# RRr89/Shared_SIMD_Scan

Measured on AMD Instinct MI355X. Metric: scanned values/sec + achieved HBM GB/s, 1e9 x 9-bit column (equality scan, bitmap + hit count out), higher is better.
Workload: dtype u32; 1 GPU; scan_eq ONE 1e+09x9bit column in 1 row-range shard(s) of <= 1000000000 rows, column=mod5, key=3; rows_total=1000000000, bits=9, parallelism=row-range shards x1

## Files before the change

shared_simd_scan_amd/csrc/kernels/in_list.hpp:

```cpp
#pragma once

#include "scan.hpp"

namespace mi355 {

template <int C, int AUX_, int VPL>
__global__ __launch_bounds__(kBlockThreads) void in_kernel(ScanArgs a)
{
    using G = ScanGeom<C, VPL>;
    constexpr int WORDS = G::WORDS;
    constexpr int AUX = AUX_ & 15;
    constexpr int NTS = store_policy_of(AUX_);
    constexpr bool BITSET = C <= 16;
    constexpr int SET_BYTES = BITSET ? ((1 << (C < 16 ? C : 16)) + 7) / 8 : 16;
    __shared__ __attribute__((aligned(16))) uint8_t lds[kWavesPerBlock][G::LDS_BYTES];
    __shared__ __attribute__((aligned(16))) uint32_t set_words[(SET_BYTES + 3) / 4];
    __shared__ __attribute__((aligned(16))) uint8_t mlds[kWavesPerBlock][1024];

    const int lane = threadIdx.x & 63;
    const int wave = __builtin_amdgcn_readfirstlane(threadIdx.x >> 6);
    uint8_t *lds_wave = lds[wave];
    const TileCtx<C, VPL> tc(a.n);
    const uint64_t stride = (uint64_t)gridDim.x * kWavesPerBlock;
    uint64_t tile = (uint64_t)blockIdx.x * kWavesPerBlock + wave;
// ... 69 lines not shown
            for (int j = 0; j < WORDS; j++) res[j] = m[j];
        }
        const uint32_t inv = a.invert;
#pragma unroll
        for (int j = 0; j < WORDS; j++) res[j] ^= inv;
        if (tile < tc.nfull) {
            if (a.and_mask) {
#pragma unroll
                for (int j = 0; j < WORDS; j++) res[j] &= mcur[j];
            }
#pragma unroll
            for (int j = 0; j < WORDS; j++) hits += __builtin_popcount(res[j]);
            prev = tile;
        } else {
            const int64_t left = (int64_t)(tc.n - tile * G::TILE_VALUES) - (int64_t)lane * VPL;
            const int nbytes = left <= 0 ? 0 : (int)((left >= VPL ? VPL : left) + 7) / 8;
            if (a.and_mask) {
                const uint8_t *mp = a.and_mask + tile * G::BITMAP_BYTES + lane * (WORDS * 4);
#pragma unroll
                for (int j = 0; j < WORDS; j++) {
                    uint32_t mm = 0;
#pragma unroll
                    for (int b = 0; b < 4; b++)
                        if (4 * j + b < nbytes) mm |= (uint32_t)mp[4 * j + b] << (8 * b);
                    res[j] &= mm;
                }
            }
            hits += tc.finish_tail(tile, res, out_lane + tile * G::BITMAP_BYTES, 1, lane);
            prev = ~0ull;
        }
        tile = next;
    }
    if (prev != ~0ull) store_words<WORDS, NTS>(out_lane + prev * G::BITMAP_BYTES, res);
    if (a.hits) hits_add(a, 0, wave_sum(hits), lane);
    hits_finalize(a, 1, lane);
}

}
```

shared_simd_scan_amd/csrc/kernels/scan.hpp:

```cpp
#pragma once

#include "tile.hpp"

namespace mi355 {

template <int C, int VPL> struct TileCtx {
    using G = ScanGeom<C, VPL>;
    uint64_t n, ntiles, nfull, data_bytes;
    uint32_t llc_inv, llc_lim;
    __device__ __forceinline__ TileCtx(uint64_t n_, uint32_t llc_inv_ = 0, uint32_t llc_lim_ = 0) : n(n_), llc_inv(llc_inv_), llc_lim(llc_lim_)
    {
        ntiles = (n + G::TILE_VALUES - 1) / G::TILE_VALUES;
        nfull = n / G::TILE_VALUES;
        data_bytes = (n * C + 7) / 8;
    }
    template <int AUX> __device__ __forceinline__ void issue(const uint8_t *packed, uint64_t t, uint8_t *lds_wave, int lane) const
    {
        if constexpr (AUX != 0) {
            if (llc_inv != 0 && (uint32_t)((t * G::TILE_BYTES) >> kLlcGranuleShift) * llc_inv <= llc_lim) {
                issue_as<0>(packed, t, lds_wave, lane);
                return;
            }
        }
        issue_as<AUX>(packed, t, lds_wave, lane);
// ... 172 lines not shown
                    for (int j = 0; j < WORDS; j++) {
                        hits += __builtin_popcount(r1[0][j]);
                        res[k][j] = r1[0][j];
                    }
                    nfull_here = k + 1;
                } else {
                    if (mask) {
                        const uint8_t *mp = mask + tile * G::BITMAP_BYTES + lane * (WORDS * 4);
                        const int64_t left = (int64_t)(tc.n - tile * G::TILE_VALUES) - (int64_t)lane * VPL;
                        const int nbytes = left <= 0 ? 0 : (int)((left >= VPL ? VPL : left) + 7) / 8;
#pragma unroll
                        for (int j = 0; j < WORDS; j++) {
                            uint32_t m = 0;
#pragma unroll
                            for (int b = 0; b < 4; b++)
                                if (4 * j + b < nbytes) m |= (uint32_t)mp[4 * j + b] << (8 * b);
                            r1[0][j] = combine(r1[0][j], m);
                        }
                    }
                    hits += tc.finish_tail(tile, r1[0], out_lane + tile * G::BITMAP_BYTES, 1, lane, store);
                }
            }
        }
        pend_chunk = chunk;
        pend_n = nfull_here;
        chunk += stride;
    }
    if (pend_n && store) {
        uint8_t *dst = out_lane + pend_chunk * K * G::BITMAP_BYTES;
#pragma unroll
        for (int q = 0; q < K; q++)
            if (q < pend_n) store_words<WORDS, NTS>(dst + q * G::BITMAP_BYTES, res[q]);
    }
    if (a.hits) hits_add(a, 0, wave_sum(hits), lane);
    hits_finalize(a, 1, lane);
}

template <int C, int AUX_, int VPL>
__global__ __launch_bounds__(kBlockThreads, (burst_occ<C, VPL, 1>() > 1 ? burst_occ<C, VPL, 1>() / 2 : 1)) void scan2_kernel(ScanArgs a)
{
    using G = ScanGeom<C, VPL>;
    constexpr int WORDS = G::WORDS;
    constexpr int AUX = AUX_ & 15;
    constexpr int NTS = store_policy_of(AUX_);
    __shared__ __attribute__((aligned(16))) uint8_t lds[kWavesPerBlock][2][G::LDS_BYTES];

    const int lane = threadIdx.x & 63;
    const int wave = __builtin_amdgcn_readfirstlane(threadIdx.x >> 6);
    uint8_t *lds1 = lds[wave][0], *lds2 = lds[wave][1];
    const TileCtx<C, VPL> tc(a.n);
    const uint64_t stride = (uint64_t)gridDim.x * kWavesPerBlock;
    uint64_t tile = (uint64_t)blockIdx.x * kWavesPerBlock + wave;
    const uint32_t k1[kMaxKeysPerPass] = {a.key[0], a.key[1], 0, 0, 0, 0, 0, 0};
    const uint32_t k2[kMaxKeysPerPass] = {a.key2[0], a.key2[1], 0, 0, 0, 0, 0, 0};
    const uint32_t inv1 = a.invert, inv2 = a.invert2, mop = a.mask_op;
    auto combine = [mop](uint32_t p2, uint32_t p1) -> uint32_t {
        return mop == 0 ? (p2 & p1) : mop == 1 ? (p2 | p1) : mop == 2 ? (p2 ^ p1) : (p1 & ~p2);
    };
    uint32_t hits = 0;
    uint8_t *const out_lane = a.out + lane * (WORDS * 4);
    const bool store = a.out != nullptr;
    uint32_t res[WORDS];
    uint64_t prev = ~0ull;

    auto issue = [&](uint64_t t) {
        tc.template issue<AUX>(a.packed, t, lds1, lane);
        tc.template issue<AUX>(a.packed2, t, lds2, lane);
    };
    if (tile < tc.ntiles) issue(tile);
    while (tile < tc.ntiles) {
        asm volatile("s_waitcnt vmcnt(0)" ::: "memory");
        uint32_t w1[G::LANE_DWORDS], w2[G::LANE_DWORDS];
        read_lane_data<C, VPL>(lds1, lane, w1);
        read_lane_data<C, VPL>(lds2, lane, w2);
        asm volatile("s_waitcnt lgkmcnt(0)" ::: "memory");
        if (prev != ~0ull && store) store_words<WORDS, NTS>(out_lane + prev * G::BITMAP_BYTES, res);
        const uint64_t next = tile + stride;
        if (next < tc.ntiles) issue(next);
        uint32_t r1[1][WORDS], r2[1][WORDS];
        decode_words<C, VPL, 0, 1, kModeRange, G::LANE_DWORDS>(w1, r1, k1);
        decode_words<C, VPL, 0, 1, kModeRange, G::LANE_DWORDS>(w2, r2, k2);
#pragma unroll
        for (int j = 0; j < WORDS; j++) res[j] = combine(r2[0][j] ^ inv2, r1[0][j] ^ inv1);
        if (tile < tc.nfull) {
#pragma unroll
            for (int j = 0; j < WORDS; j++) hits += __builtin_popcount(res[j]);
            prev = tile;
        } else {
            hits += tc.finish_tail(tile, res, out_lane + tile * G::BITMAP_BYTES, 1, lane, store);
            prev = ~0ull;
        }
        tile = next;
    }
    if (prev != ~0ull && store) store_words<WORDS, NTS>(out_lane + prev * G::BITMAP_BYTES, res);
    if (a.hits) hits_add(a, 0, wave_sum(hits), lane);
    hits_finalize(a, 1, lane);
}

__device__ __forceinline__ void transpose4x4_bytes(const uint32_t (&r)[4], uint32_t (&c)[4])
{
    const uint32_t t0 = __builtin_amdgcn_perm(r[1], r[0], 0x05010400u);
    const uint32_t t1 = __builtin_amdgcn_perm(r[1], r[0], 0x07030602u);
    const uint32_t t2 = __builtin_amdgcn_perm(r[3], r[2], 0x05010400u);
    const uint32_t t3 = __builtin_amdgcn_perm(r[3], r[2], 0x07030602u);
    c[0] = __builtin_amdgcn_perm(t2, t0, 0x05040100u);
    c[1] = __builtin_amdgcn_perm(t2, t0, 0x07060302u);
    c[2] = __builtin_amdgcn_perm(t3, t1, 0x05040100u);
    c[3] = __builtin_amdgcn_perm(t3, t1, 0x07060302u);
}

}
```

shared_simd_scan_amd/csrc/kernels/shared.hpp:

```cpp
#pragma once

#include "scan.hpp"

namespace mi355 {

template <int C, int AUX_, int VPL>
__global__ __launch_bounds__(kBlockThreads) void shared_general_kernel(ScanArgs a)
{
    using G = ScanGeom<C, VPL>;
    constexpr int NK = kMaxKeysPerPass;
    constexpr int WORDS = G::WORDS;
    constexpr int AUX = AUX_ & 15;
    __shared__ __attribute__((aligned(16))) uint8_t lds[kWavesPerBlock][G::LDS_BYTES];
    __shared__ uint32_t s_hits[kMaxKeys];
    block_hits_clear(s_hits);
    __syncthreads();

    const int lane = threadIdx.x & 63;
    const int wave = __builtin_amdgcn_readfirstlane(threadIdx.x >> 6);
    uint8_t *lds_wave = lds[wave];
    const TileCtx<C, VPL> tc(a.n);
    const uint64_t stride = (uint64_t)gridDim.x * kWavesPerBlock;
    uint64_t tile = (uint64_t)blockIdx.x * kWavesPerBlock + wave;
    const uint32_t P = a.nkeys;
// ... 45 lines not shown
#pragma unroll
                        for (int j = 0; j < WORDS; j++) cnt += __builtin_popcount(res[q][j]);
                    }
                    cnts[q] = cnt;
                }
            }
            if (a.hits) block_hits_add8(s_hits, pass * kMaxKeysPerPass, P, cnts, lane);
            if (a.layout != 0 && full) {
                const uint32_t nk = (P - pass * 8) < 8 ? (P - pass * 8) : 8;
                const uint64_t g0 = tile * G::BITMAP_BYTES + (uint64_t)lane * (WORDS * 4);
#pragma unroll
                for (int j = 0; j < WORDS; j++) {
                    const uint32_t r0[4] = {res[0][j], res[1][j], res[2][j], res[3][j]};
                    const uint32_t r1[4] = {res[4][j], res[5][j], res[6][j], res[7][j]};
                    uint32_t c0[4], c1[4];
                    transpose4x4_bytes(r0, c0);
                    transpose4x4_bytes(r1, c1);
#pragma unroll
                    for (int b = 0; b < 4; b++) {
                        uint8_t *dst = a.out + (g0 + 4 * j + b) * P + pass * 8;
                        if (nk == 8) {
                            store8_unaligned(dst, c0[b], c1[b]);
                        } else {
#pragma unroll
                            for (int q = 0; q < 8; q++)
                                if ((uint32_t)q < nk) dst[q] = (uint8_t)((q < 4 ? c0[b] : c1[b]) >> (8 * (q & 3)));
                        }
                    }
                }
            }
        }
        tile = next;
    }
    if (a.hits) block_hits_flush(a, s_hits, P);
    hits_finalize(a, P, lane);
}

template <int C, int AUX_, int VPL>
__global__ __launch_bounds__(kBlockThreads) void shared_pair_kernel(ScanArgs a)
{
    using G = ScanGeom<C, VPL>;
    constexpr int WORDS = G::WORDS;
    constexpr int AUX = AUX_ & 15;
    constexpr int NTS = store_policy_of(AUX_);
    __shared__ __attribute__((aligned(16))) uint8_t lds[kWavesPerBlock][G::LDS_BYTES];
    const int lane = threadIdx.x & 63;
    const int wave = __builtin_amdgcn_readfirstlane(threadIdx.x >> 6);
    uint8_t *lds_wave = lds[wave];
    const TileCtx<C, VPL> tc(a.n);
    const uint64_t stride = (uint64_t)gridDim.x * kWavesPerBlock;
    uint64_t tile = (uint64_t)blockIdx.x * kWavesPerBlock + wave;
    const uint32_t k0 = a.key[0], k1 = a.key[1];
    const bool linear = a.layout != 0;
    uint32_t hits0 = 0, hits1 = 0;

    if (tile < tc.ntiles) tc.template issue<AUX>(a.packed, tile, lds_wave, lane);
    int behind = 0;
    while (tile < tc.ntiles) {
        if (behind == 2)
            asm volatile("s_waitcnt vmcnt(2)" ::: "memory");
        else if (behind == 1)
            asm volatile("s_waitcnt vmcnt(1)" ::: "memory");
        else
            asm volatile("s_waitcnt vmcnt(0)" ::: "memory");
        uint32_t w[G::LANE_DWORDS];
        read_lane_data<C, VPL>(lds_wave, lane, w);
        asm volatile("s_waitcnt lgkmcnt(0)" ::: "memory");
        const uint64_t next = tile + stride;
// ... 8 lines not shown
            for (int j = 0; j < WORDS; j++) {
                hits0 += __builtin_popcount(r0[0][j]);
                hits1 += __builtin_popcount(r1[0][j]);
            }
            if (!linear) {
                uint8_t *dst = a.out + tile * G::BITMAP_BYTES + lane * (WORDS * 4);
                store_words<WORDS, NTS>(dst, r0[0]);
                store_words<WORDS, NTS>(dst + a.out_stride, r1[0]);
                behind = 2;
            } else {
                uint32_t y[2 * WORDS];
#pragma unroll
                for (int j = 0; j < WORDS; j++) {
                    y[2 * j] = __builtin_amdgcn_perm(r1[0][j], r0[0][j], 0x05010400u);
                    y[2 * j + 1] = __builtin_amdgcn_perm(r1[0][j], r0[0][j], 0x07030602u);
                }
                uint8_t *dst = a.out + (tile * G::BITMAP_BYTES + (uint64_t)lane * (WORDS * 4)) * 2;
#pragma unroll
                for (int i = 0; i < 2 * WORDS; i += 4) {
                    const uint32_t v[4] = {y[i], y[i + 1], y[i + 2], y[i + 3]};
                    store_words<4, NTS>(dst + 4 * i, v);
                }
                behind = WORDS / 2;
            }
        } else {
            uint8_t *dst = linear ? a.out + (tile * G::BITMAP_BYTES + (uint64_t)lane * (WORDS * 4)) * 2
                                  : a.out + tile * G::BITMAP_BYTES + lane * (WORDS * 4);
            hits0 += tc.finish_tail(tile, r0[0], dst, linear ? 2 : 1, lane);
            hits1 += tc.finish_tail(tile, r1[0], linear ? dst + 1 : dst + a.out_stride, linear ? 2 : 1, lane);
            behind = 0;
        }
        tile = next;
    }
    if (a.hits) {
        hits_add(a, 0, wave_sum(hits0), lane);
        hits_add(a, 1, wave_sum(hits1), lane);
    }
    hits_finalize(a, 2, lane);
}


struct __attribute__((packed, aligned(1))) Unaligned128 { uint32_t w[4]; };

extern __shared__ __attribute__((aligned(16))) uint8_t mi355_dyn_lds[];

template <int C, bool MULTI> struct LutGeom {
    static constexpr int ND = MULTI ? (C <= 10 ? 1 : (C + 7) / 8) : (C <= 16 ? 1 : (C <= 24 ? 2 : 3));
    static constexpr bool SINGLE = ND == 1;
    static constexpr int DIGIT_BITS = SINGLE ? C : (MULTI ? 8 : (C + ND - 1) / ND);
    static constexpr int ENTRIES = 1 << DIGIT_BITS;
    static constexpr int TABLE_BYTES = ND * ENTRIES;
    static __device__ __forceinline__ uint32_t digit(uint32_t x, int d)
    {
        return (d == ND - 1) ? (x >> (DIGIT_BITS * d)) : ((x >> (DIGIT_BITS * d)) & (uint32_t)(ENTRIES - 1));
    }
};

__device__ __forceinline__ void transpose8x8(uint32_t &lo, uint32_t &hi)
{
    uint32_t t;
    t = (lo ^ (lo >> 7)) & 0x00AA00AAu;  lo ^= t ^ (t << 7);
    t = (hi ^ (hi >> 7)) & 0x00AA00AAu;  hi ^= t ^ (t << 7);
    t = (lo ^ (lo >> 14)) & 0x0000CCCCu; lo ^= t ^ (t << 14);
    t = (hi ^ (hi >> 14)) & 0x0000CCCCu; hi ^= t ^ (t << 14);
    t = (lo ^ ((lo >> 28) | (hi << 4))) & 0xF0F0F0F0u;
    lo ^= t;
    hi ^= t >> 4;
}

template <int C, bool MULTI> __device__ __forceinline__ uint32_t lut_lookup(const uint8_t *table, uint32_t x)
{
// ... 403 lines not shown
                } else {
                    lut_words<C, VPL, true, MULTI>(xs, table, valid, out);
                }
                uint32_t tcnt[8];
#pragma unroll
                for (int q = 0; q < 8; q++) {
                    const uint32_t k = pass * 8 + q;
                    tcnt[q] = 0;
                    if (k < P) {
                        uint32_t cnt = 0;
#pragma unroll
                        for (int j = 0; j < WORDS; j++) cnt += __builtin_popcount(out[q][j]);
                        if constexpr (!MULTI)
                            hits[q] += cnt;
                        else
                            tcnt[q] = cnt;
                        uint8_t *dst = LAYOUT == 0
                                           ? a.out + (uint64_t)k * a.out_stride + tile * G::BITMAP_BYTES + lane * (WORDS * 4)
                                           : a.out + (tile * G::BITMAP_BYTES + (uint64_t)lane * GROUPS) * P + k;
                        const uint64_t bstride = LAYOUT == 0 ? 1 : P;
#pragma unroll
                        for (int b = 0; b < WORDS * 4; b++)
                            if (b < nbytes) dst[(uint64_t)b * bstride] = (uint8_t)(out[q][b >> 2] >> (8 * (b & 3)));
                    }
                }
                if constexpr (MULTI) {
                    if (a.hits) block_hits_add8(s_hits, pass * 8, P, tcnt, lane);
                }
            }
        }
        tile = next;
    }
    if constexpr (MULTI) {
        if (a.hits) block_hits_flush(a, s_hits, P);
    }
    if constexpr (!MULTI) {
        if (prev != ~0ull) {
            if (lin8) {
                u32x4 staged[GROUPS / 2];
                stage_get(staged);
                stage_store(prev, staged);
            } else {
                store_full(prev, 0, resp);
            }
        }
        if (a.hits) {
#pragma unroll
            for (int q = 0; q < 8; q++) {
                uint32_t s = wave_sum(hits[q]);
                if ((uint32_t)q < P) hits_add(a, q, s, lane);
            }
        }
    }
    hits_finalize(a, P, lane);
}

template <int C, bool BIG = false> struct WideLutGeom {
    static constexpr int ND = C <= 10 ? 1 : (BIG && C >= 17 && C <= 20) ? 2 : (BIG && C >= 25 && C <= 30) ? 3 : (C + 7) / 8;
    static constexpr bool SINGLE = ND == 1;
    static constexpr int DIGIT_BITS = SINGLE ? C : (BIG ? (C + ND - 1) / ND : 8);
    static constexpr int ENTRIES = 1 << DIGIT_BITS;
    static constexpr int TABLE_DWORDS = ND * ENTRIES;
    static constexpr int TABLE_BYTES = TABLE_DWORDS * 4;
    static __device__ __forceinline__ uint32_t digit(uint32_t x, int d)
    {
        return (d == ND - 1) ? (x >> (DIGIT_BITS * d)) : ((x >> (DIGIT_BITS * d)) & (uint32_t)(ENTRIES - 1));
    }
    static __device__ __forceinline__ uint32_t lookup(const uint32_t *table, uint32_t x)
    {
        if constexpr (SINGLE) {
            return table[x];
        } else {
            uint32_t m = table[digit(x, 0)];
#pragma unroll
            for (int d = 1; d < ND; d++) m &= table[d * ENTRIES + digit(x, d)];
            return m;
        }
    }
};

__device__ __forceinline__ void wait_dma_behind_stores(uint32_t nstores)
{
    if (nstores >= 48)
        asm volatile("s_waitcnt vmcnt(48)" ::: "memory");
    else if (nstores >= 32)
        asm volatile("s_waitcnt vmcnt(32)" ::: "memory");
    else if (nstores >= 16)
// ... 142 lines not shown
                        }
                        if (a.hits) block_hits_add8(s_hits, pass * 8, P, cnt, lane);
                        if (full) {
                            if constexpr (LAYOUT == 0) {
                                uint8_t *dst = a.out + (uint64_t)(pass * 8) * a.out_stride + tile * G::BITMAP_BYTES + lane * (WORDS * 4);
#pragma unroll
                                for (int q = 0; q < 8; q++) {
                                    if (pass * 8 + q < P) store_words<WORDS, NTS>(dst, out[q]);
                                    dst += a.out_stride;
                                }
                            }
                        } else {
                            const int nbytes = (valid + 7) / 8;
#pragma unroll
                            for (int q = 0; q < 8; q++) {
                                const uint32_t k = pass * 8 + q;
                                if (k < P) {
                                    uint8_t *dst = LAYOUT == 0
                                                       ? a.out + (uint64_t)k * a.out_stride + tile * G::BITMAP_BYTES + lane * (WORDS * 4)
                                                       : a.out + (tile * G::BITMAP_BYTES + (uint64_t)lane * GROUPS) * P + k;
                                    const uint64_t bstride = LAYOUT == 0 ? 1 : P;
#pragma unroll
                                    for (int bb = 0; bb < WORDS * 4; bb++)
                                        if (bb < nbytes) dst[(uint64_t)bb * bstride] = (uint8_t)(out[q][bb >> 2] >> (8 * (bb & 3)));
                                }
                            }
                        }
                    }
                }
            }
        }
        tile = next;
    }
    if (a.hits) block_hits_flush(a, s_hits, P);
    hits_finalize(a, P, lane);
}

constexpr uint32_t kPackedFlushTiles = 512;

template <int C, int AUX_, int VPL, int RC = 0, bool BIG = false>
__global__ __launch_bounds__(kBlockThreads) void shared_wide2_kernel(ScanArgs a)
{
    using G = ScanGeom<C, VPL>;
    using L = WideLutGeom<C, BIG>;
    constexpr bool REGCNT = RC == 1;
    constexpr int WORDS = G::WORDS;
    constexpr int AUX = AUX_ & 15;
    constexpr int NTS = store_policy_of(AUX_);
    __shared__ __attribute__((aligned(16))) uint8_t lds[kWavesPerBlock][G::LDS_BYTES];
    __shared__ uint32_t s_hits[kMaxKeys];
    constexpr bool HIST = C <= 12;
    __shared__ uint32_t hist[HIST ? (1 << C) : 1];
    uint32_t *const lut = (uint32_t *)mi355_dyn_lds;
    block_hits_clear(s_hits);
    if constexpr (HIST)
        for (uint32_t k = threadIdx.x; k < (1u << C); k += kBlockThreads) hist[k] = 0;

    const int lane = threadIdx.x & 63;
    const int wave = __builtin_amdgcn_readfirstlane(threadIdx.x >> 6);
    uint8_t *lds_wave = lds[wave];
    const TileCtx<C, VPL> tc(a.n);
    const uint64_t stride = (uint64_t)gridDim.x * kWavesPerBlock;
    uint64_t tile = (uint64_t)blockIdx.x * kWavesPerBlock + wave;
    const uint32_t P = a.nkeys;
    const uint32_t npass32 = (P + 31) / 32;
    constexpr bool reg_counts = REGCNT;
    const bool use_hist = HIST && P >= 64 && RC == 0;
    uint32_t acc[REGCNT ? 4 : 1][8];
// ... 461 lines not shown
            if (copy_out) image_store(pend_gal, pend_a0, pend_end, iv, ihb, itb);
            pend_end = 0;
            if (staged) {
                const uint32_t first = s * row_step;
                const uint32_t rows_in_step = first >= rows_here ? 0u : (rows_here - first < row_step ? rows_here - first : row_step);
                if (rows_in_step) {
                    pend_gal = step_g0 - step_a0;
                    pend_a0 = step_a0;
                    pend_end = step_a0 + rows_in_step * P;
                }
            }
        }
        asm volatile("s_waitcnt lgkmcnt(0)" ::: "memory");
        const uint64_t next = tile + stride;
        if (next < tc.ntiles) tc.template issue<AUX>(a.packed, next, lds_wave, lane);
        tile = next;
    }
    if (pend_end) {
        u32x4 iv[3];
        uint32_t ihb = 0, itb = 0;
        image_load(pend_a0, pend_end, iv, ihb, itb);
        image_store(pend_gal, pend_a0, pend_end, iv, ihb, itb);
    }
    if (!use_hist && a.hits) flush_counts();
    if constexpr (HIST) {
        if (a.hits && use_hist) {
            __syncthreads();
            for (uint32_t k = threadIdx.x; k < P; k += kBlockThreads) {
                const uint32_t key = (uint32_t)a.keys_dev[k];
                s_hits[k] = (key >> C) == 0 ? hist[key] : 0u;
            }
        }
    }
    if (a.hits) block_hits_flush(a, s_hits, P);
    hits_finalize(a, P, lane);
}

template <int C, int AUX_>
__global__ __launch_bounds__(kBlockThreads) void shared_linear2_kernel(ScanArgs a)
{
    constexpr int VPL = 64;
    using G = ScanGeom<C, VPL>;
    using L = WideLutGeom<C>;
    constexpr int AUX = AUX_ & 15;
    constexpr int ROWS = G::TILE_VALUES / 8;
    constexpr int ROW_DW = (C + 3) / 4;
    constexpr int LOAD_DW = (C + 3 + 3) / 4;
    __shared__ __attribute__((aligned(16))) uint8_t lds[kWavesPerBlock][G::LDS_BYTES + 16];
    __shared__ uint32_t s_hits[kMaxKeys];
    constexpr bool HIST = C <= 12;
    __shared__ uint32_t hist[HIST ? (1 << C) : 1];
    uint32_t *const lut = (uint32_t *)mi355_dyn_lds;
    block_hits_clear(s_hits);
    if constexpr (HIST)
        for (uint32_t k = threadIdx.x; k < (1u << C); k += kBlockThreads) hist[k] = 0;

    const int lane = threadIdx.x & 63;
    const int wave = __builtin_amdgcn_readfirstlane(threadIdx.x >> 6);
    uint8_t *lds_wave = lds[wave];
    const TileCtx<C, VPL> tc(a.n);
    const uint64_t stride = (uint64_t)gridDim.x * kWavesPerBlock;
    uint64_t tile = (uint64_t)blockIdx.x * kWavesPerBlock + wave;
    const uint32_t P = a.nkeys;
    const uint32_t Tf = P / 32, R = P % 32;
    const uint32_t T = Tf + (R ? 1u : 0u);
    const bool attached = R != 0 && (Tf == 1 || (Tf >= 2 && (a.flags & kSetShortAttached)));
    const bool dedicated = R != 0 && !attached;
    const bool aligned16 = (P & 15u) == 0;
// ... 168 lines not shown
                                __hip_atomic_fetch_add(&hist[x[i]], 1u, __ATOMIC_RELAXED, __HIP_MEMORY_SCOPE_WORKGROUP);
                    }
                }
            }
            if (count_packed) {
                if (++since_f == 31) flush(cbf, 32u * quarter, since_f);
                if (attached && ++since_s == 31) flush(cbs, 32u * Tf, since_s);
            }
            if (dedicated) {
                const uint32_t covered = (s + 1) * rows_per_step;
                while (64u * (short_done + 1) <= covered && short_done < (uint32_t)ROWS / 64u) short_step(short_done++);
            }
        }
        if (dedicated)
            while (short_done < (uint32_t)ROWS / 64u) short_step(short_done++);
        asm volatile("s_waitcnt lgkmcnt(0)" ::: "memory");
        const uint64_t next = tile + stride;
        if (next < tc.ntiles) tc.template issue<AUX>(a.packed, next, lds_wave, lane);
        tile = next;
    }
    if (count_packed) {
        if (has_table) flush(cbf, 32u * quarter, since_f);
        if (R != 0) flush(cbs, 32u * Tf, since_s);
    }
    if constexpr (HIST) {
        if (a.hits && use_hist) {
            __syncthreads();
            for (uint32_t k = threadIdx.x; k < P; k += kBlockThreads) {
                const uint32_t key = (uint32_t)a.keys_dev[k];
                s_hits[k] = (key >> C) == 0 ? hist[key] : 0u;
            }
        }
    }
    if (a.hits) block_hits_flush(a, s_hits, P);
    hits_finalize(a, P, lane);
}


template <int C, int BASE, int N, int K, int NW> __device__ __forceinline__ void extract_range(const uint32_t (&w)[NW], uint32_t (&x)[N])
{
    x[K] = extract<C, BASE + K, NW>(w);
    if constexpr (K + 1 < N) extract_range<C, BASE, N, K + 1, NW>(w, x);
}

template <int C, int AUX_, int RC, bool BIG>
__global__ __launch_bounds__(kBlockThreads, ((RC == 0 || C <= 10) ? 3 : 2)) void shared_wide3_kernel(ScanArgs a)
{
    constexpr int VPL = 64;
    using G = ScanGeom<C, VPL>;
    using L = WideLutGeom<C, BIG>;
    constexpr int WORDS = G::WORDS;
    constexpr int AUX = AUX_ & 15;
    constexpr int NTS = store_policy_of(AUX_);
    __shared__ __attribute__((aligned(16))) uint8_t lds[kWavesPerBlock][G::LDS_BYTES];
    uint32_t *const lut = (uint32_t *)mi355_dyn_lds;

    const int lane = threadIdx.x & 63;
    const int wave = __builtin_amdgcn_readfirstlane(threadIdx.x >> 6);
    uint8_t *lds_wave = lds[wave];
    const TileCtx<C, VPL> tc(a.n);
    const uint64_t stride = (uint64_t)gridDim.x * kWavesPerBlock;
    uint64_t tile = (uint64_t)blockIdx.x * kWavesPerBlock + wave;
    const uint32_t P = a.nkeys;
    const uint32_t npass32 = (P + 31) / 32;

    if (tile < tc.ntiles) tc.template issue<AUX>(a.packed, tile, lds_wave, lane);
    for (uint32_t i = threadIdx.x; i < npass32 * L::TABLE_DWORDS; i += kBlockThreads) lut[i] = 0;
    __syncthreads();
// ... 361 lines not shown
```

shared_simd_scan_amd/csrc/kernels/tile.hpp:

```cpp
#pragma once

#include <hip/hip_runtime.h>
#include <stdint.h>

#include "../switches.hpp"

namespace mi355 {

typedef uint32_t u32x4 __attribute__((ext_vector_type(4)));
typedef uint32_t u32x2 __attribute__((ext_vector_type(2)));

#define MI355_GPTR(p) ((const __attribute__((address_space(1))) void *)(p))
#define MI355_LPTR(p) ((__attribute__((address_space(3))) void *)(p))

constexpr int kWavesPerBlock = 4;
constexpr int kBlockThreads = kWavesPerBlock * 64;
constexpr int kCuLdsBytes = 160 * 1024;
constexpr int kMaxKeysPerPass = 8;
constexpr uint64_t value_reach(unsigned c, uint64_t count) { return (c < 32 && count > (1ull << c)) ? (1ull << c) : count; }
constexpr int kMaxKeys = 1024;

template <int C, int VPL> struct ScanGeom {
    static_assert(VPL == 32 || VPL == 64 || VPL == 128, "VPL");
    static constexpr int WORDS = VPL / 32;
    static constexpr int LANE_DWORDS = VPL * C / 32;
    static constexpr int LANE_BYTES = LANE_DWORDS * 4;
    static constexpr int TILE_VALUES = 64 * VPL;
    static constexpr int TILE_BYTES = 64 * LANE_BYTES;
    static constexpr int DMA_INSTRS = (TILE_BYTES + 1023) / 1024;
    static constexpr int LDS_BYTES = DMA_INSTRS * 1024;
    static constexpr int BITMAP_BYTES = TILE_VALUES / 8;
    static constexpr int OCC_LDS = kCuLdsBytes / (4 * LDS_BYTES + 64);
    static constexpr int OCC = OCC_LDS >= 8 ? 8 : (OCC_LDS < 1 ? 1 : OCC_LDS);
};

enum ScanMode { kModeEq = 0, kModeRange = 1, kModeShared = 2 };

template <int C> constexpr int narrow_k() { return C == 1 ? 8 : (C <= 3 ? 4 : (C <= 5 ? 3 : (C <= 7 ? 2 : 0))); }
// ... 315 lines not shown
    return v >= 32 ? 0xffffffffu : (v <= 0 ? 0u : ((1u << v) - 1u));
}

struct __attribute__((packed, aligned(1))) Unaligned64 { uint32_t lo, hi; };
__device__ __forceinline__ void store8_unaligned(uint8_t *dst, uint32_t lo, uint32_t hi)
{
    Unaligned64 v;
    v.lo = lo;
    v.hi = hi;
    *(Unaligned64 *)dst = v;
}

constexpr int store_policy_of(int aux) { return (aux & 32) ? 2 : ((aux & 16) ? 1 : 0); }

template <int WORDS, int NT = 0> __device__ __forceinline__ void store_words(uint8_t *dst, const uint32_t (&v)[WORDS])
{
    if constexpr (WORDS == 4) {
        u32x4 t = {v[0], v[1], v[2], v[3]};
        if constexpr (NT == 2) {
            asm volatile("global_store_dwordx4 %0, %1, off sc1" ::"v"(dst), "v"(t) : "memory");
        } else if constexpr (NT == 1) __builtin_nontemporal_store(t, (u32x4 *)dst); else *(u32x4 *)dst = t;
    } else if constexpr (WORDS == 2) {
        u32x2 t = {v[0], v[1]};
        if constexpr (NT == 2) {
            asm volatile("global_store_dwordx2 %0, %1, off sc1" ::"v"(dst), "v"(t) : "memory");
        } else if constexpr (NT == 1) __builtin_nontemporal_store(t, (u32x2 *)dst); else *(u32x2 *)dst = t;
    } else {
        if constexpr (NT) __builtin_nontemporal_store(v[0], (uint32_t *)dst); else *(uint32_t *)dst = v[0];
    }
}

constexpr int kHitSlots = 64;
constexpr int kDoneGroups = 16;
constexpr int kScratchWords = kHitSlots * kMaxKeys + 8 + kDoneGroups * 16;
constexpr int kScratchDone = kHitSlots * kMaxKeys;
constexpr int kScratchGroupDone = kScratchDone + 8;

__device__ __forceinline__ void hits_add(const ScanArgs &a, uint32_t k, uint32_t wave_total, int lane)
{
    if (lane == 0 && wave_total)
        __hip_atomic_fetch_add(a.scratch + (blockIdx.x % kHitSlots) * kMaxKeys + k, (unsigned long long)wave_total,
                               __ATOMIC_RELAXED, __HIP_MEMORY_SCOPE_AGENT);
}

__device__ __forceinline__ void hits_finalize(const ScanArgs &a, uint32_t P, int lane)
{
    if (!a.hits) return;
    __shared__ uint32_t s_last;
    asm volatile("s_waitcnt vmcnt(0)" ::: "memory");
    __syncthreads();
    if (threadIdx.x == 0) {
        const uint32_t g = blockIdx.x % kDoneGroups;
        const uint32_t in_group = (gridDim.x - g + kDoneGroups - 1) / kDoneGroups;
        const uint32_t ngroups = gridDim.x < (unsigned)kDoneGroups ? gridDim.x : (unsigned)kDoneGroups;
        unsigned long long *const gdone = a.scratch + kScratchGroupDone + g * 16;
        uint32_t last = 0;
        if (__hip_atomic_fetch_add(gdone, 1ull, __ATOMIC_RELAXED, __HIP_MEMORY_SCOPE_AGENT) == (unsigned long long)in_group - 1) {
            __hip_atomic_store(gdone, 0ull, __ATOMIC_RELAXED, __HIP_MEMORY_SCOPE_AGENT);
            last = __hip_atomic_fetch_add(a.scratch + kScratchDone, 1ull, __ATOMIC_RELAXED, __HIP_MEMORY_SCOPE_AGENT) == (unsigned long long)ngroups - 1;
        }
        s_last = last;
    }
    __syncthreads();
    if (s_last) {
        const uint32_t nslots = gridDim.x < (unsigned)kHitSlots ? gridDim.x : (unsigned)kHitSlots;
        if (P <= 16u) {
            for (uint32_t k = threadIdx.x >> 6; k < P; k += kBlockThreads / 64) {
                const unsigned long long v = (uint32_t)lane < nslots
                                                 ? __hip_atomic_exchange(a.scratch + (uint32_t)lane * kMaxKeys + k, 0ull, __ATOMIC_RELAXED, __HIP_MEMORY_SCOPE_AGENT)
                                                 : 0ull;
                const unsigned long long lo = wave_sum((uint32_t)(v & 0xffffffull)), mid = wave_sum((uint32_t)((v >> 24) & 0xffffffull)),
                                         hi = wave_sum((uint32_t)(v >> 48));
                if (lane == 0) a.hits[k] = lo + (mid << 24) + (hi << 48);
            }
            if (threadIdx.x == 0) __hip_atomic_store(a.scratch + kScratchDone, 0ull, __ATOMIC_RELAXED, __HIP_MEMORY_SCOPE_AGENT);
            return;
        }
        for (uint32_t k = threadIdx.x; k < P; k += kBlockThreads) {
            unsigned long long v = 0;
#pragma unroll 8
            for (uint32_t sl = 0; sl < nslots; sl++)
                v += __hip_atomic_exchange(a.scratch + sl * kMaxKeys + k, 0ull, __ATOMIC_RELAXED, __HIP_MEMORY_SCOPE_AGENT);
            a.hits[k] = v;
        }
        if (threadIdx.x == 0) __hip_atomic_store(a.scratch + kScratchDone, 0ull, __ATOMIC_RELAXED, __HIP_MEMORY_SCOPE_AGENT);
    }
}

__device__ __forceinline__ void block_hits_clear(uint32_t *s_hits)
{
    for (uint32_t k = threadIdx.x; k < (uint32_t)kMaxKeys; k += kBlockThreads) s_hits[k] = 0;
}
__device__ __forceinline__ void block_hits_add8(uint32_t *s_hits, uint32_t kbase, uint32_t P, const uint32_t (&cnt)[8], int lane)
{
    uint32_t p0 = cnt[0] | (cnt[1] << 16), p1 = cnt[2] | (cnt[3] << 16), p2 = cnt[4] | (cnt[5] << 16), p3 = cnt[6] | (cnt[7] << 16);
    p0 = wave_sum(p0);
    p1 = wave_sum(p1);
    p2 = wave_sum(p2);
    p3 = wave_sum(p3);
    if (lane == 0) {
        const uint32_t v[8] = {p0 & 0xffff, p0 >> 16, p1 & 0xffff, p1 >> 16, p2 & 0xffff, p2 >> 16, p3 & 0xffff, p3 >> 16};
#pragma unroll
        for (int q = 0; q < 8; q++)
            if (kbase + q < P && v[q]) atomicAdd(&s_hits[kbase + q], v[q]);
    }
}

__device__ __forceinline__ void block_hits_flush(const ScanArgs &a, uint32_t *s_hits, uint32_t P)
{
    __syncthreads();
    for (uint32_t k = threadIdx.x; k < P; k += blockDim.x) {
        const uint32_t v = s_hits[k];
        if (v)
            __hip_atomic_fetch_add(a.scratch + (blockIdx.x % kHitSlots) * kMaxKeys + k, (unsigned long long)v, __ATOMIC_RELAXED,
                                   __HIP_MEMORY_SCOPE_AGENT);
    }
}

template <int C, int LK, int J, int GI, int NW>
__device__ __forceinline__ void narrow_step(const uint32_t (&w)[NW], uint32_t &acc, const uint8_t *table)
{
    constexpr int FIRST = LK * GI;
    constexpr int LEN = (32 - FIRST) < LK ? (32 - FIRST) : LK;
    uint32_t m = table[extract_at<(32 * J + FIRST) * C, LEN * C, NW>(w)];
    if constexpr (LEN < LK) m &= (1u << LEN) - 1u;
    acc = (acc << LEN) | m;
    if constexpr (GI > 0) narrow_step<C, LK, J, GI - 1, NW>(w, acc, table);
}

template <int C, int VPL, int LK, int J, int NW>
__device__ __forceinline__ void decode_words_narrow(const uint32_t (&w)[NW], uint32_t (&res)[1][VPL / 32], const uint8_t *table)
{
    uint32_t acc = 0;
    narrow_step<C, LK, J, (32 + LK - 1) / LK - 1, NW>(w, acc, table);
    res[0][J] = acc;
    if constexpr (J + 1 < VPL / 32) decode_words_narrow<C, VPL, LK, J + 1, NW>(w, res, table);
}

}
```

shared_simd_scan_amd/csrc/predicates/columns.hpp:

```cpp
#pragma once

#include "../kernels.hpp"
#include "../kernels/rt_column.hpp"

namespace mi355 {

struct ColumnsArgs {
    ScanArgs s;
    uint32_t c2;
    uint32_t nts;
    uint32_t lo, span;
    int64_t lo64;
    uint64_t span64;
};

constexpr int kColumnsMaskLds = 1024;

constexpr int columns_vpl(int C, bool same) { return same ? scan_vpl(C, kModeRange) : 32; }
template <int C1, int VPL, bool SAME> constexpr uint32_t columns_wave_lds(uint32_t c2)
{
    return (uint32_t)ScanGeom<C1, VPL>::LDS_BYTES + (SAME ? 1u : 2u) * ((64u * VPL * c2 / 8 + 1023u) / 1024u * 1024u) + (uint32_t)kColumnsMaskLds;
}
template <int C1, int VPL, bool SAME> constexpr uint32_t columns_block_lds(uint32_t c2)
{
// ... 138 lines not shown
            lds2 = lds2_next;
            lds2_next = t2;
        }
#pragma unroll
        for (int j = 0; j < WORDS; j++) res[j] ^= inv;
        if (full) {
            if (mask) {
#pragma unroll
                for (int j = 0; j < WORDS; j++) res[j] = combine(res[j], mw[j]);
            }
#pragma unroll
            for (int j = 0; j < WORDS; j++) hits += __builtin_popcount(res[j]);
            prev = tile;
        } else {
            if (mask) {
                const uint8_t *mp = mask + tile * MASK_TILE + lane * (WORDS * 4);
                const int64_t left = (int64_t)(tc.n - tile * G::TILE_VALUES) - (int64_t)lane * VPL;
                const int nbytes = left <= 0 ? 0 : (int)((left >= VPL ? VPL : left) + 7) / 8;
#pragma unroll
                for (int j = 0; j < WORDS; j++) {
                    uint32_t m = 0;
#pragma unroll
                    for (int b = 0; b < 4; b++)
                        if (4 * j + b < nbytes) m |= (uint32_t)mp[4 * j + b] << (8 * b);
                    res[j] = combine(res[j], m);
                }
            }
            hits += tc.finish_tail(tile, res, out_lane + tile * G::BITMAP_BYTES, 1, lane, store);
            prev = ~0ull;
        }
        tile = next;
    }
    if (prev != ~0ull && store) store_prev();
    if (s.hits) hits_add(s, 0, wave_sum(hits), lane);
    hits_finalize(s, 1, lane);
}

}
```

shared_simd_scan_amd/csrc/predicates/where.hpp:

```cpp
#pragma once

#include "../kernels.hpp"

namespace mi355 {

struct WhereArgs {
    ScanArgs s;
    uint32_t lo[kMaxKeysPerPass], span[kMaxKeysPerPass], neg[kMaxKeysPerPass];
    const uint32_t *preds_dev;
};

template <int C> struct WhereLutGeom {
    static_assert(C >= 1 && C <= 16, "full tables: c <= 16");
    static constexpr int ENTRIES = 1 << C;
    static constexpr int TABLE_BYTES = ENTRIES < 4 ? 4 : ENTRIES;
    static constexpr int TABLE_DWORDS = TABLE_BYTES / 4;
    static constexpr int CH = TABLE_DWORDS >= 4 ? 4 : 1;
    static constexpr int T = TABLE_DWORDS / CH;
};

template <int C, bool MULTI>
__device__ __forceinline__ void where_build_tables(const WhereArgs &a, uint8_t *lut, uint32_t P, uint32_t npass, uint32_t *s_carry)
{
    using W = WhereLutGeom<C>;
// ... 328 lines not shown
                } else {
                    lut_words<C, VPL, true, false>(xs, table, valid, out);
                }
                uint32_t tcnt[8];
#pragma unroll
                for (int q = 0; q < 8; q++) {
                    const uint32_t k = pass * 8 + q;
                    tcnt[q] = 0;
                    if (k < P) {
                        uint32_t cnt = 0;
#pragma unroll
                        for (int j = 0; j < WORDS; j++) cnt += __builtin_popcount(out[q][j]);
                        if constexpr (!MULTI)
                            hits[q] += cnt;
                        else
                            tcnt[q] = cnt;
                        uint8_t *dst = LAYOUT == 0
                                           ? s.out + (uint64_t)k * s.out_stride + tile * G::BITMAP_BYTES + lane * (WORDS * 4)
                                           : s.out + (tile * G::BITMAP_BYTES + (uint64_t)lane * GROUPS) * P + k;
                        const uint64_t bstride = LAYOUT == 0 ? 1 : P;
#pragma unroll
                        for (int b = 0; b < WORDS * 4; b++)
                            if (b < nbytes) dst[(uint64_t)b * bstride] = (uint8_t)(out[q][b >> 2] >> (8 * (b & 3)));
                    }
                }
                if constexpr (MULTI) {
                    if (s.hits) block_hits_add8(s_hits, pass * 8, P, tcnt, lane);
                }
            }
        }
        tile = next;
    }
    if constexpr (MULTI) {
        if (s.hits) block_hits_flush(s, s_hits, P);
    }
    if constexpr (!MULTI) {
        if (prev != ~0ull) {
            if (lin8) {
                u32x4 staged[GROUPS / 2];
                stage_get(staged);
                stage_store(prev, staged);
            } else {
                store_full(prev, 0, resp);
            }
        }
        if (s.hits) {
#pragma unroll
            for (int q = 0; q < 8; q++) {
                uint32_t t = wave_sum(hits[q]);
                if ((uint32_t)q < P) hits_add(s, q, t, lane);
            }
        }
    }
    hits_finalize(s, P, lane);
}

__device__ __forceinline__ void push_range4(uint32_t &a0, uint32_t &a1, uint32_t &a2, uint32_t &a3, uint32_t x, uint32_t l0, uint32_t l1,
                                            uint32_t l2, uint32_t l3, uint32_t s0, uint32_t s1, uint32_t s2, uint32_t s3)
{
    unsigned long long m0, m1, m2, m3;
    uint32_t t0, t1, t2, t3;
    asm("v_subrev_u32_e32 %8, %13, %12\n\t"
        "v_subrev_u32_e32 %9, %14, %12\n\t"
        "v_subrev_u32_e32 %10, %15, %12\n\t"
        "v_subrev_u32_e32 %11, %16, %12\n\t"
        "v_cmp_ge_u32_e64 %4, %17, %8\n\t"
        "v_cmp_ge_u32_e64 %5, %18, %9\n\t"
        "v_cmp_ge_u32_e64 %6, %19, %10\n\t"
        "v_cmp_ge_u32_e64 %7, %20, %11\n\t"
        "v_addc_co_u32_e64 %0, %4, %0, %0, %4\n\t"
        "v_addc_co_u32_e64 %1, %5, %1, %1, %5\n\t"
        "v_addc_co_u32_e64 %2, %6, %2, %2, %6\n\t"
        "v_addc_co_u32_e64 %3, %7, %3, %3, %7"
        : "+v"(a0), "+v"(a1), "+v"(a2), "+v"(a3), "=&s"(m0), "=&s"(m1), "=&s"(m2), "=&s"(m3), "=&v"(t0), "=&v"(t1), "=&v"(t2),
          "=&v"(t3)
        : "v"(x), "s"(l0), "s"(l1), "s"(l2), "s"(l3), "s"(s0), "s"(s1), "s"(s2), "s"(s3));
}

template <int C, int J, int K, int NW>
__device__ __forceinline__ void where_step8(const uint32_t (&w)[NW], uint32_t (&acc)[8], const uint32_t (&lo)[8], const uint32_t (&span)[8])
{
    const uint32_t x = extract<C, 32 * J + K, NW>(w);
    push_range4(acc[0], acc[1], acc[2], acc[3], x, lo[0], lo[1], lo[2], lo[3], span[0], span[1], span[2], span[3]);
    push_range4(acc[4], acc[5], acc[6], acc[7], x, lo[4], lo[5], lo[6], lo[7], span[4], span[5], span[6], span[7]);
    if constexpr (K > 0) where_step8<C, J, K - 1, NW>(w, acc, lo, span);
}

// ... 86 lines not shown
#pragma unroll
                        for (int j = 0; j < WORDS; j++) cnt += __builtin_popcount(res[q][j]);
                    }
                    cnts[q] = cnt;
                }
            }
            if (s.hits) block_hits_add8(s_hits, pass * NK, P, cnts, lane);
            if (s.layout != 0 && full) {
                const uint32_t nk = (P - pass * 8) < 8 ? (P - pass * 8) : 8;
                const uint64_t g0 = tile * G::BITMAP_BYTES + (uint64_t)lane * (WORDS * 4);
#pragma unroll
                for (int j = 0; j < WORDS; j++) {
                    const uint32_t r0[4] = {res[0][j], res[1][j], res[2][j], res[3][j]};
                    const uint32_t r1[4] = {res[4][j], res[5][j], res[6][j], res[7][j]};
                    uint32_t c0[4], c1[4];
                    transpose4x4_bytes(r0, c0);
                    transpose4x4_bytes(r1, c1);
#pragma unroll
                    for (int b = 0; b < 4; b++) {
                        uint8_t *dst = s.out + (g0 + 4 * j + b) * P + pass * 8;
                        if (nk == 8) {
                            store8_unaligned(dst, c0[b], c1[b]);
                        } else {
#pragma unroll
                            for (int q = 0; q < 8; q++)
                                if ((uint32_t)q < nk) dst[q] = (uint8_t)((q < 4 ? c0[b] : c1[b]) >> (8 * (q & 3)));
                        }
                    }
                }
            }
        }
        tile = next;
    }
    if (s.hits) block_hits_flush(s, s_hits, P);
    hits_finalize(s, P, lane);
}

}
```

shared_simd_scan_amd/csrc/semijoin/semijoin.hpp:

```cpp
#pragma once

#include "../kernels.hpp"

namespace mi355 {

struct SemiArgs {
    ScanArgs s;
    const uint8_t *set;
    uint32_t set_bytes;
    uint32_t limit;
    uint32_t last_keep;
};

constexpr uint32_t kSemiMaskLds = 1024;
constexpr uint32_t kSemiLdsSlack = 64;
constexpr int kSemiGlobalMinBits = 20;

template <int C> constexpr uint32_t semijoin_static_lds()
{
    return (uint32_t)kWavesPerBlock * ((uint32_t)ScanGeom<C, scan_vpl(C, kModeEq)>::LDS_BYTES + kSemiMaskLds);
}
constexpr uint64_t semijoin_lds_max_bits()
{
    constexpr uint32_t widest = semijoin_static_lds<32>() > semijoin_static_lds<16>() ? semijoin_static_lds<32>() : semijoin_static_lds<16>();
// ... 120 lines not shown
                res[j] = acc;
            }
        }
#pragma unroll
        for (int j = 0; j < WORDS; j++) res[j] ^= inv;
        if (tile < tc.nfull) {
            if (mask) {
#pragma unroll
                for (int j = 0; j < WORDS; j++) res[j] &= mcur[j];
            }
#pragma unroll
            for (int j = 0; j < WORDS; j++) hits += __builtin_popcount(res[j]);
            prev = tile;
        } else {
            if (mask) {
                const int64_t left = (int64_t)(tc.n - tile * G::TILE_VALUES) - (int64_t)lane * VPL;
                const int nbytes = left <= 0 ? 0 : (int)((left >= VPL ? VPL : left) + 7) / 8;
                const uint8_t *mp = mask + tile * G::BITMAP_BYTES + lane * (WORDS * 4);
#pragma unroll
                for (int j = 0; j < WORDS; j++) {
                    uint32_t mm = 0;
#pragma unroll
                    for (int q = 0; q < 4; q++)
                        if (4 * j + q < nbytes) mm |= (uint32_t)mp[4 * j + q] << (8 * q);
                    res[j] &= mm;
                }
            }
            hits += tc.finish_tail(tile, res, out_lane + tile * G::BITMAP_BYTES, 1, lane, store);
            prev = ~0ull;
        }
        tile = next;
    }
    if (prev != ~0ull && store) store_words<WORDS, NTS>(out_lane + prev * G::BITMAP_BYTES, res);
    if (a.s.hits) hits_add(a.s, 0, wave_sum(hits), lane);
    hits_finalize(a.s, 1, lane);
}

template <int C, int AUX_> __device__ __forceinline__ void semijoin_first_tile(const SemiArgs &a, uint8_t *lds_wave, uint8_t *mlds_wave)
{
    constexpr int VPL = scan_vpl(C, kModeEq);
    using G = ScanGeom<C, VPL>;
    const int lane = threadIdx.x & 63;
    const int wave = __builtin_amdgcn_readfirstlane(threadIdx.x >> 6);
    const TileCtx<C, VPL> tc(a.s.n);
    const uint64_t tile = (uint64_t)blockIdx.x * kWavesPerBlock + wave;
    if (tile >= tc.ntiles) return;
    if (a.s.and_mask && tile < tc.nfull && lane * 16 < G::BITMAP_BYTES)
        __builtin_amdgcn_global_load_lds(MI355_GPTR(a.s.and_mask + tile * G::BITMAP_BYTES + lane * 16), MI355_LPTR(mlds_wave), 16, 0, 0);
    tc.template issue<AUX_ & 15>(a.s.packed, tile, lds_wave, lane);
}

template <int C, int AUX_> __global__ __launch_bounds__(kBlockThreads) void semijoin_lds_kernel(SemiArgs a)
{
    using G = ScanGeom<C, scan_vpl(C, kModeEq)>;
    __shared__ __attribute__((aligned(16))) uint8_t lds[kWavesPerBlock][G::LDS_BYTES];
    __shared__ __attribute__((aligned(16))) uint8_t mlds[kWavesPerBlock][kSemiMaskLds];
    const int wave = __builtin_amdgcn_readfirstlane(threadIdx.x >> 6);
    semijoin_first_tile<C, AUX_>(a, lds[wave], mlds[wave]);
    const uint8_t *const set_lds = semijoin_stage_set(a);
    semijoin_tiles<C, AUX_, true>(a, set_lds, lds[wave], mlds[wave]);
}

template <int C, int AUX_> __global__ __launch_bounds__(kBlockThreads) void semijoin_global_kernel(SemiArgs a)
{
    static_assert(C >= kSemiGlobalMinBits, "narrower columns reach no set beyond the LDS tier");
    using G = ScanGeom<C, scan_vpl(C, kModeEq)>;
    __shared__ __attribute__((aligned(16))) uint8_t lds[kWavesPerBlock][G::LDS_BYTES];
    __shared__ __attribute__((aligned(16))) uint8_t mlds[kWavesPerBlock][kSemiMaskLds];
// ... 7 lines not shown
```

Measured before the change: 5275 billion values/s.

## Fuse hit-count reduction into packed ticket+sum atomics with group tree

Replaces the per-wave hit atomic adds plus the separate done-counter finalize step with a block-level LDS reduction. Each block then does one atomic per key that packs a completion ticket and the running hit sum into a 64-bit word, combined through a two-level group tree. The last block in each group forwards the group total, and the last group writes the final count. This is meant to cut the number of global atomics, barriers and the extra finalize round trip at kernel end, at the cost of limits on key count, block count and row count. It falls back to the old path when those limits are exceeded.

Result: no change. 5328 billion values/s (median of 3 runs) (+1.0%).

```diff
diff --git a/shared_simd_scan_amd/csrc/kernels/hits_word.hpp b/shared_simd_scan_amd/csrc/kernels/hits_word.hpp
--- /dev/null
+++ b/shared_simd_scan_amd/csrc/kernels/hits_word.hpp
@@ -0,0 +1,30 @@
+#pragma once
+
+#include <stdint.h>
+
+namespace mi355 {
+
+constexpr int kHitWordHitBits = 48;
+constexpr int kHitWordTicketBits = 16;
+constexpr int kHitWordKeys = 16;
+constexpr int kHitWordGroups = 16;
+constexpr uint64_t kHitWordHitMask = (1ull << kHitWordHitBits) - 1;
+constexpr uint64_t kHitWordMaxTickets = (1ull << kHitWordTicketBits) - 1;
+
+constexpr uint64_t hit_word_pack(uint64_t tickets, uint64_t hits) { return (tickets << kHitWordHitBits) | hits; }
+constexpr uint64_t hit_word_hits(uint64_t w) { return w & kHitWordHitMask; }
+constexpr uint64_t hit_word_tickets(uint64_t w) { return w >> kHitWordHitBits; }
+
+constexpr uint64_t hit_word_add(uint64_t hits) { return hit_word_pack(1, hits); }
+constexpr bool hit_word_completes(uint64_t old, uint64_t members) { return hit_word_tickets(old) + 1 == members; }
+constexpr uint64_t hit_word_total(uint64_t old, uint64_t hits) { return hit_word_hits(old) + hits; }
+
+constexpr uint64_t hit_groups(uint64_t blocks) { return blocks < (uint64_t)kHitWordGroups ? blocks : (uint64_t)kHitWordGroups; }
+constexpr uint64_t hit_group_size(uint64_t blocks, uint64_t g) { return (blocks - g + kHitWordGroups - 1) / kHitWordGroups; }
+
+constexpr bool hit_word_applies(uint64_t keys, uint64_t blocks, uint64_t rows)
+{
+    return keys >= 1 && keys <= (uint64_t)kHitWordKeys && blocks >= 1 && hit_group_size(blocks, 0) <= kHitWordMaxTickets && rows <= kHitWordHitMask;
+}
+
+}
diff --git a/shared_simd_scan_amd/csrc/kernels/in_list.hpp b/shared_simd_scan_amd/csrc/kernels/in_list.hpp
--- a/shared_simd_scan_amd/csrc/kernels/in_list.hpp
+++ b/shared_simd_scan_amd/csrc/kernels/in_list.hpp
@@ -125,8 +125,7 @@
         tile = next;
     }
     if (prev != ~0ull) store_words<WORDS, NTS>(out_lane + prev * G::BITMAP_BYTES, res);
-    if (a.hits) hits_add(a, 0, wave_sum(hits), lane);
-    hits_finalize(a, 1, lane);
+    hits_finish1(a, hits, lane);
 }
 
 }
diff --git a/shared_simd_scan_amd/csrc/kernels/scan.hpp b/shared_simd_scan_amd/csrc/kernels/scan.hpp
--- a/shared_simd_scan_amd/csrc/kernels/scan.hpp
+++ b/shared_simd_scan_amd/csrc/kernels/scan.hpp
@@ -228,8 +228,7 @@
         for (int q = 0; q < K; q++)
             if (q < pend_n) store_words<WORDS, NTS>(dst + q * G::BITMAP_BYTES, res[q]);
     }
-    if (a.hits) hits_add(a, 0, wave_sum(hits), lane);
-    hits_finalize(a, 1, lane);
+    hits_finish1(a, hits, lane);
 }
 
 template <int C, int AUX_, int VPL>
@@ -289,8 +288,7 @@
         tile = next;
     }
     if (prev != ~0ull && store) store_words<WORDS, NTS>(out_lane + prev * G::BITMAP_BYTES, res);
-    if (a.hits) hits_add(a, 0, wave_sum(hits), lane);
-    hits_finalize(a, 1, lane);
+    hits_finish1(a, hits, lane);
 }
 
 __device__ __forceinline__ void transpose4x4_bytes(const uint32_t (&r)[4], uint32_t (&c)[4])
diff --git a/shared_simd_scan_amd/csrc/kernels/shared.hpp b/shared_simd_scan_amd/csrc/kernels/shared.hpp
--- a/shared_simd_scan_amd/csrc/kernels/shared.hpp
+++ b/shared_simd_scan_amd/csrc/kernels/shared.hpp
@@ -101,8 +101,7 @@
         }
         tile = next;
     }
-    if (a.hits) block_hits_flush(a, s_hits, P);
-    hits_finalize(a, P, lane);
+    block_hits_finish(a, s_hits, P, lane);
 }
 
 template <int C, int AUX_, int VPL>
@@ -177,11 +176,8 @@
         }
         tile = next;
     }
-    if (a.hits) {
-        hits_add(a, 0, wave_sum(hits0), lane);
-        hits_add(a, 1, wave_sum(hits1), lane);
-    }
-    hits_finalize(a, 2, lane);
+    const uint32_t hits01[2] = {hits0, hits1};
+    hits_finish<2>(a, 2, hits01, lane);
 }
 
 
@@ -651,7 +647,7 @@
         tile = next;
     }
     if constexpr (MULTI) {
-        if (a.hits) block_hits_flush(a, s_hits, P);
+        block_hits_finish(a, s_hits, P, lane);
     }
     if constexpr (!MULTI) {
         if (prev != ~0ull) {
@@ -663,15 +659,8 @@
                 store_full(prev, 0, resp);
             }
         }
-        if (a.hits) {
-#pragma unroll
-            for (int q = 0; q < 8; q++) {
-                uint32_t s = wave_sum(hits[q]);
-                if ((uint32_t)q < P) hits_add(a, q, s, lane);
-            }
-        }
-    }
-    hits_finalize(a, P, lane);
+        hits_finish<8>(a, P, hits, lane);
+    }
 }
 
 template <int C, bool BIG = false> struct WideLutGeom {
@@ -880,8 +869,7 @@
         }
         tile = next;
     }
-    if (a.hits) block_hits_flush(a, s_hits, P);
-    hits_finalize(a, P, lane);
+    block_hits_finish(a, s_hits, P, lane);
 }
 
 constexpr uint32_t kPackedFlushTiles = 512;
@@ -1409,8 +1397,7 @@
             }
         }
     }
-    if (a.hits) block_hits_flush(a, s_hits, P);
-    hits_finalize(a, P, lane);
+    block_hits_finish(a, s_hits, P, lane);
 }
 
 template <int C, int AUX_>
@@ -1645,8 +1632,7 @@
             }
         }
     }
-    if (a.hits) block_hits_flush(a, s_hits, P);
-    hits_finalize(a, P, lane);
+    block_hits_finish(a, s_hits, P, lane);
 }
 
 
diff --git a/shared_simd_scan_amd/csrc/kernels/tile.hpp b/shared_simd_scan_amd/csrc/kernels/tile.hpp
--- a/shared_simd_scan_amd/csrc/kernels/tile.hpp
+++ b/shared_simd_scan_amd/csrc/kernels/tile.hpp
@@ -4,6 +4,7 @@
 #include <stdint.h>
 
 #include "../switches.hpp"
+#include "hits_word.hpp"
 
 namespace mi355 {
 
@@ -385,9 +386,11 @@
 
 constexpr int kHitSlots = 64;
 constexpr int kDoneGroups = 16;
-constexpr int kScratchWords = kHitSlots * kMaxKeys + 8 + kDoneGroups * 16;
 constexpr int kScratchDone = kHitSlots * kMaxKeys;
 constexpr int kScratchGroupDone = kScratchDone + 8;
+constexpr int kScratchTop = kScratchGroupDone + kDoneGroups * 16;
+constexpr int kScratchWords = kScratchTop + kHitWordKeys;
+static_assert(kDoneGroups == kHitWordGroups && kHitWordKeys == 16, "a group's 128-byte line holds its 16 key words");
 
 __device__ __forceinline__ void hits_add(const ScanArgs &a, uint32_t k, uint32_t wave_total, int lane)
 {
@@ -396,10 +399,10 @@
                                __ATOMIC_RELAXED, __HIP_MEMORY_SCOPE_AGENT);
 }
 
-__device__ __forceinline__ void hits_finalize(const ScanArgs &a, uint32_t P, int lane)
+__device__ __forceinline__ void hits_finalize_at(const ScanArgs &a, uint32_t P, int lane, uint32_t *s_last_p)
 {
     if (!a.hits) return;
-    __shared__ uint32_t s_last;
+    uint32_t &s_last = *s_last_p;
     asm volatile("s_waitcnt vmcnt(0)" ::: "memory");
     __syncthreads();
     if (threadIdx.x == 0) {
@@ -439,6 +442,68 @@
         if (threadIdx.x == 0) __hip_atomic_store(a.scratch + kScratchDone, 0ull, __ATOMIC_RELAXED, __HIP_MEMORY_SCOPE_AGENT);
     }
 }
+__device__ __forceinline__ void hits_finalize(const ScanArgs &a, uint32_t P, int lane)
+{
+    __shared__ uint32_t s_last;
+    hits_finalize_at(a, P, lane, &s_last);
+}
+
+__device__ __forceinline__ bool hits_fused(const ScanArgs &a, uint32_t P) { return hit_word_applies(P, gridDim.x, a.n); }
+
+__device__ __forceinline__ void hits_publish(const ScanArgs &a, uint32_t k, unsigned long long block_hits)
+{
+    const uint32_t g = blockIdx.x % kDoneGroups;
+    unsigned long long *const gword = a.scratch + kScratchGroupDone + g * kHitWordKeys + k;
+    const unsigned long long gold = __hip_atomic_fetch_add(gword, (unsigned long long)hit_word_add(block_hits), __ATOMIC_RELAXED, __HIP_MEMORY_SCOPE_AGENT);
+    if (!hit_word_completes(gold, hit_group_size(gridDim.x, g))) return;
+    const unsigned long long group_total = hit_word_total(gold, block_hits);
+    __hip_atomic_store(gword, 0ull, __ATOMIC_RELAXED, __HIP_MEMORY_SCOPE_AGENT);
+    unsigned long long *const tword = a.scratch + kScratchTop + k;
+    const unsigned long long told = __hip_atomic_fetch_add(tword, (unsigned long long)hit_word_add(group_total), __ATOMIC_RELAXED, __HIP_MEMORY_SCOPE_AGENT);
+    if (!hit_word_completes(told, hit_groups(gridDim.x))) return;
+    a.hits[k] = hit_word_total(told, group_total);
+    __hip_atomic_store(tword, 0ull, __ATOMIC_RELAXED, __HIP_MEMORY_SCOPE_AGENT);
+}
+
+__device__ __forceinline__ void lds_barrier()
+{
+    asm volatile("s_waitcnt lgkmcnt(0)\n\ts_barrier" ::: "memory");
+}
+
+template <int NQ>
+__device__ __forceinline__ void hits_finish(const ScanArgs &a, uint32_t P, const uint32_t (&lane_hits)[NQ], int lane)
+{
+    static_assert(NQ <= kHitWordKeys, "NQ");
+    if (!a.hits) return;
+    __shared__ uint32_t s_wave[kWavesPerBlock][NQ];
+    uint32_t total[NQ];
+#pragma unroll
+    for (int q = 0; q < NQ; q++) total[q] = wave_sum(lane_hits[q]);
+    if (!hits_fused(a, P)) {
+#pragma unroll
+        for (int q = 0; q < NQ; q++)
+            if ((uint32_t)q < P) hits_add(a, q, total[q], lane);
+        hits_finalize_at(a, P, lane, &s_wave[0][0]);
+        return;
+    }
+    if (lane == 0) {
+#pragma unroll
+        for (int q = 0; q < NQ; q++) s_wave[threadIdx.x >> 6][q] = total[q];
+    }
+    lds_barrier();
+    if (threadIdx.x < (NQ < P ? NQ : P)) {
+        unsigned long long v = 0;
+#pragma unroll
+        for (int w = 0; w < kWavesPerBlock; w++) v += s_wave[w][threadIdx.x];
+        hits_publish(a, threadIdx.x, v);
+    }
+}
+
+__device__ __forceinline__ void hits_finish1(const ScanArgs &a, uint32_t lane_hits, int lane)
+{
+    const uint32_t one[1] = {lane_hits};
+    hits_finish<1>(a, 1, one, lane);
+}
 
 __device__ __forceinline__ void block_hits_clear(uint32_t *s_hits)
 {
@@ -470,6 +535,18 @@
     }
 }
 
+__device__ __forceinline__ void block_hits_finish(const ScanArgs &a, uint32_t *s_hits, uint32_t P, int lane)
+{
+    if (!a.hits) return;
+    if (!hits_fused(a, P)) {
+        block_hits_flush(a, s_hits, P);
+        hits_finalize(a, P, lane);
+        return;
+    }
+    lds_barrier();
+    if (threadIdx.x < P) hits_publish(a, threadIdx.x, s_hits[threadIdx.x]);
+}
+
 template <int C, int LK, int J, int GI, int NW>
 __device__ __forceinline__ void narrow_step(const uint32_t (&w)[NW], uint32_t &acc, const uint8_t *table)
 {
diff --git a/shared_simd_scan_amd/csrc/predicates/columns.hpp b/shared_simd_scan_amd/csrc/predicates/columns.hpp
--- a/shared_simd_scan_amd/csrc/predicates/columns.hpp
+++ b/shared_simd_scan_amd/csrc/predicates/columns.hpp
@@ -194,8 +194,7 @@
         tile = next;
     }
     if (prev != ~0ull && store) store_prev();
-    if (s.hits) hits_add(s, 0, wave_sum(hits), lane);
-    hits_finalize(s, 1, lane);
-}
-
-}
+    hits_finish1(s, hits, lane);
+}
+
+}
diff --git a/shared_simd_scan_amd/csrc/predicates/where.hpp b/shared_simd_scan_amd/csrc/predicates/where.hpp
--- a/shared_simd_scan_amd/csrc/predicates/where.hpp
+++ b/shared_simd_scan_amd/csrc/predicates/where.hpp
@@ -384,7 +384,7 @@
         tile = next;
     }
     if constexpr (MULTI) {
-        if (s.hits) block_hits_flush(s, s_hits, P);
+        block_hits_finish(s, s_hits, P, lane);
     }
     if constexpr (!MULTI) {
         if (prev != ~0ull) {
@@ -396,15 +396,8 @@
                 store_full(prev, 0, resp);
             }
         }
-        if (s.hits) {
-#pragma unroll
-            for (int q = 0; q < 8; q++) {
-                uint32_t t = wave_sum(hits[q]);
-                if ((uint32_t)q < P) hits_add(s, q, t, lane);
-            }
-        }
+        hits_finish<8>(s, P, hits, lane);
     }
-    hits_finalize(s, P, lane);
 }
 
 __device__ __forceinline__ void push_range4(uint32_t &a0, uint32_t &a1, uint32_t &a2, uint32_t &a3, uint32_t x, uint32_t l0, uint32_t l1,
@@ -557,8 +550,7 @@
         }
         tile = next;
     }
-    if (s.hits) block_hits_flush(s, s_hits, P);
-    hits_finalize(s, P, lane);
-}
-
-}
+    block_hits_finish(s, s_hits, P, lane);
+}
+
+}
diff --git a/shared_simd_scan_amd/csrc/semijoin/semijoin.hpp b/shared_simd_scan_amd/csrc/semijoin/semijoin.hpp
--- a/shared_simd_scan_amd/csrc/semijoin/semijoin.hpp
+++ b/shared_simd_scan_amd/csrc/semijoin/semijoin.hpp
@@ -176,8 +176,7 @@
         tile = next;
     }
     if (prev != ~0ull && store) store_words<WORDS, NTS>(out_lane + prev * G::BITMAP_BYTES, res);
-    if (a.s.hits) hits_add(a.s, 0, wave_sum(hits), lane);
-    hits_finalize(a.s, 1, lane);
+    hits_finish1(a.s, hits, lane);
 }
 
 template <int C, int AUX_> __device__ __forceinline__ void semijoin_first_tile(const SemiArgs &a, uint8_t *lds_wave, uint8_t *mlds_wave)
```
